# jianwen-xie/Latent-Space-Normalizing-Flow

Hardware: NVIDIA B200
Metric: langevin_latent_steps_per_sec (higher is better)
Workload: dtype fp16-hi/lo-3pass-fwd+bf16-hi/lo-3pass-bwd/f32-accumulate (fp32-equivalent)

## Files before the change

include/lsnf.h:

```cpp
#ifndef LSNF_H_
#define LSNF_H_

#include <stddef.h>
#include <stdint.h>

#ifdef __cplusplus
extern "C" {
#endif

#define LSNF_ABI_VERSION 1

typedef struct lsnf_plan lsnf_plan;
typedef void* lsnf_stream;

typedef enum lsnf_status {
  LSNF_OK = 0,
  LSNF_ERR_INVALID = -1,
  LSNF_ERR_CUDA = -2,
  LSNF_ERR_STATE = -3,
  LSNF_ERR_UNSUPPORTED = -4
} lsnf_status;

typedef enum lsnf_arch {
  LSNF_ARCH_NONE = -1,
// ... 112 lines not shown
  int32_t out_off_y[LSNF_MAX_PHASES], out_off_x[LSNF_MAX_PHASES];
  int32_t out_phase_split;
  int32_t out_channels;
  int32_t epilogue;
  int32_t k_splits;
  int32_t a_planes;
  int32_t a_h, a_w;
  int32_t tap_gen_k;
  int32_t b_k;
  int32_t b_rows;
  int32_t operand_fp16;
  int32_t passes;
  int64_t a_offset, b_offset, out_offset;
  int64_t flops;
} lsnf_stage_info;

int lsnf_plan_num_stages(const lsnf_plan* plan);
int lsnf_plan_stage_info(const lsnf_plan* plan, int32_t index, lsnf_stage_info* out);
int lsnf_plan_pack_index(const lsnf_plan* plan, int32_t index, int32_t ci, int32_t co, int32_t ky, int32_t kx,
                         int64_t* row, int64_t* col);

#define LSNF_KERNEL_SINGLE 0
#define LSNF_KERNEL_PAIR 1
typedef struct lsnf_launch_info {
  int32_t kernel;
  int32_t grid_x, grid_y, grid_z, block;
  int32_t ring_stages;
  int32_t stage_bytes;
  int32_t smem_bytes;
  int32_t ctas_per_sm;
  int32_t tmem_columns;
  int32_t tma_store;
  int32_t stream_k;
  int32_t reserved[4];
} lsnf_launch_info;
int lsnf_plan_stage_launch_info(const lsnf_plan* plan, int32_t index, int32_t num_sms, lsnf_launch_info* out);

#ifdef __cplusplus
}
#endif
#endif
```

latent-space-normalizing-flow_b200/_cabi.py:

```python
from __future__ import annotations

import ctypes as C
import os

_HERE = os.path.dirname(os.path.abspath(__file__))
LIB_PATH = os.environ.get("LSNF_LIB") or os.path.join(_HERE, "_lib", "liblsnf_b200.so")
_lib = None

LSNF_MAX_TAPS = 16
LSNF_MAX_PHASES = 4
FLOW_PTRS_PER_STEP = 12

ARCH = {"none": -1, "svhn": 0, "cifar10": 1, "celeba_crop": 2, "celeba_hq256": 3}
GEMM_TCGEN05, GEMM_SIMT = 0, 1


class Config(C.Structure):
    _fields_ = [("arch", C.c_int32), ("batch", C.c_int32), ("nz", C.c_int32), ("ngf", C.c_int32), ("nc", C.c_int32),
                ("f_depth", C.c_int32), ("f_width", C.c_int32), ("f_permutation", C.c_int32),
                ("f_coupling", C.c_int32), ("leak", C.c_float), ("gemm_impl", C.c_int32),
                ("bwd_passes", C.c_int32), ("train", C.c_int32), ("reserved", C.c_int32 * 3)]


class Tap(C.Structure):
    _fields_ = [("dy", C.c_int32), ("dx", C.c_int32), ("plane", C.c_int32), ("brow", C.c_int32)]


class StageInfo(C.Structure):
    _fields_ = [("kind", C.c_int32), ("layer", C.c_int32), ("grid_h", C.c_int32), ("grid_w", C.c_int32),
                ("box_b", C.c_int32), ("box_h", C.c_int32), ("box_w", C.c_int32), ("k_per_tap", C.c_int32),
                ("n_valid", C.c_int32), ("n_pad", C.c_int32), ("block_n", C.c_int32), ("n_phases", C.c_int32),
                ("n_taps", C.c_int32 * LSNF_MAX_PHASES), ("taps", (Tap * LSNF_MAX_TAPS) * LSNF_MAX_PHASES),
                ("out_mul", C.c_int32), ("out_off_y", C.c_int32 * LSNF_MAX_PHASES),
                ("out_off_x", C.c_int32 * LSNF_MAX_PHASES), ("out_phase_split", C.c_int32),
                ("out_channels", C.c_int32), ("epilogue", C.c_int32), ("k_splits", C.c_int32),
                ("a_planes", C.c_int32), ("a_h", C.c_int32), ("a_w", C.c_int32), ("tap_gen_k", C.c_int32),
                ("b_k", C.c_int32), ("b_rows", C.c_int32), ("operand_fp16", C.c_int32), ("passes", C.c_int32),
                ("a_offset", C.c_int64), ("b_offset", C.c_int64), ("out_offset", C.c_int64), ("flops", C.c_int64)]


class LaunchInfo(C.Structure):
    _fields_ = [("kernel", C.c_int32), ("grid_x", C.c_int32), ("grid_y", C.c_int32), ("grid_z", C.c_int32),
                ("block", C.c_int32), ("ring_stages", C.c_int32), ("stage_bytes", C.c_int32),
                ("smem_bytes", C.c_int32), ("ctas_per_sm", C.c_int32), ("tmem_columns", C.c_int32),
                ("tma_store", C.c_int32), ("stream_k", C.c_int32), ("reserved", C.c_int32 * 4)]


KERNEL_SINGLE, KERNEL_PAIR = 0, 1

EXPORTS = {
    "lsnf_abi_version": (C.c_int, []),
    "lsnf_last_error": (C.c_char_p, []),
    "lsnf_plan_create": (C.c_int, [C.POINTER(Config), C.POINTER(C.c_void_p)]),
    "lsnf_plan_destroy": (None, [C.c_void_p]),
    "lsnf_workspace_bytes": (C.c_size_t, [C.c_void_p]),
    "lsnf_plan_bind": (C.c_int, [C.c_void_p, C.c_void_p, C.c_size_t]),
    "lsnf_pack_generator_weights": (C.c_int, [C.c_void_p, C.POINTER(C.c_void_p), C.POINTER(C.c_void_p), C.c_int32,
                                              C.c_void_p]),
    "lsnf_pack_flow_weights": (C.c_int, [C.c_void_p, C.POINTER(C.c_void_p), C.POINTER(C.c_void_p),
                                         C.POINTER(C.c_void_p), C.c_void_p, C.POINTER(C.c_void_p), C.c_void_p]),
    "lsnf_generator_forward": (C.c_int, [C.c_void_p, C.c_void_p, C.c_void_p, C.c_void_p]),
    "lsnf_generator_dgrad": (C.c_int, [C.c_void_p, C.c_void_p, C.c_float, C.c_void_p, C.c_void_p]),
    "lsnf_flow_forward": (C.c_int, [C.c_void_p, C.c_void_p, C.c_void_p, C.c_void_p, C.c_void_p, C.c_void_p,
                                    C.c_void_p]),
    "lsnf_flow_inverse": (C.c_int, [C.c_void_p, C.c_void_p, C.c_void_p, C.c_void_p, C.c_void_p]),
    "lsnf_langevin_update": (C.c_int, [C.c_void_p, C.c_void_p, C.c_void_p, C.c_void_p, C.c_float, C.c_void_p,
                                       C.c_int32, C.c_uint64, C.c_uint64, C.c_uint32, C.c_void_p, C.c_void_p]),
    "lsnf_langevin_run": (C.c_int, [C.c_void_p, C.c_void_p, C.c_void_p, C.c_int32, C.c_float, C.c_float, C.c_int32,
                                    C.c_void_p, C.c_uint64, C.c_uint64, C.c_void_p, C.c_void_p, C.c_void_p]),
    "lsnf_sample_prior": (C.c_int, [C.c_void_p, C.c_void_p, C.c_void_p, C.c_void_p, C.c_int32, C.c_void_p]),
    "lsnf_generator_grad_floats": (C.c_size_t, [C.c_void_p]),
    "lsnf_generator_grad_layout": (C.c_int, [C.c_void_p, C.POINTER(C.c_int64), C.POINTER(C.c_int64)]),
    "lsnf_generator_param_grads": (C.c_int, [C.c_void_p, C.c_void_p, C.c_void_p, C.c_int32, C.c_void_p, C.c_void_p,
                                             C.c_int32, C.c_void_p]),
    "lsnf_flow_grad_floats": (C.c_size_t, [C.c_void_p]),
    "lsnf_flow_grad_layout": (C.c_int, [C.c_void_p, C.POINTER(C.c_int64), C.POINTER(C.c_int64)]),
    "lsnf_flow_param_grads": (C.c_int, [C.c_void_p, C.c_void_p, C.c_int32, C.c_void_p, C.c_void_p, C.c_void_p]),
    "lsnf_langevin_run_masked": (C.c_int, [C.c_void_p, C.c_void_p, C.c_void_p, C.c_void_p, C.c_int32, C.c_float,
# ... 53 lines not shown
```

latent-space-normalizing-flow_b200/csrc/lsnf_internal.cuh:

```cuda
#pragma once
#include <cuda.h>
#include <cuda_bf16.h>
#include <cuda_fp16.h>
#include <cuda_runtime.h>
#include <stdint.h>

#include <string>
#include <vector>

#include "lsnf.h"

namespace lsnf {

constexpr int BLOCK_M = 128;
constexpr int BLOCK_K = 64;

enum Epilogue : int32_t {
  EPI_ACT_HL = 0,
  EPI_OUT_TANH = 1,
  EPI_GRAD_HL = 2,
  EPI_PARTIAL = 3
};

struct TapDev {
  int16_t dy, dx, plane;
  int16_t bsh;
  int32_t brow;
};

struct PhaseDev {
  int32_t ntaps;
  int32_t mo, no;
  TapDev taps[LSNF_MAX_TAPS];
};

struct StageDev {
  const __nv_bfloat16* a;
  const __nv_bfloat16* b;
  int32_t aP, B, Hg, Wg, Ka, b_rows;
  int32_t aH, aW, tap_gen, b_k;
  int32_t bB, bH, bW;
  int32_t tiles_b, tiles_h, tiles_w;
  int32_t n_valid, n_pad, block_n;
  int32_t nphase, ksplit, it_per_split;
  int32_t epi, bias_mod, oC, ms, split;
  float leak;
  const float* bias;
  void* out;
  uint32_t* mbits;
  int64_t sP, sB, sH, sW, sPos;
  int32_t nc, Ho, Wo, pad_;
  int32_t fp16, out_fp16;
  int32_t passes, out_single;
  const float* descale;
  int64_t rows_total;
  float* sk_slots;
  int32_t* sk_flags;
  int32_t sk_enable;
  int32_t wgrad;
  int32_t out_tma, nst;
  PhaseDev ph[LSNF_MAX_PHASES];
};

struct StageHost {
  lsnf_stage_info info;
  StageDev dev;
  CUtensorMap tmA, tmB, tmO;
  bool maps_ready = false;
  int layer = 0;
  int kind = 0;
  int k = 0, s = 0, p = 0, ci = 0, co = 0;
  size_t a_off = 0, b_off = 0, out_off = 0, mbits_off = 0, bias_off = 0;
  size_t b_bytes = 0;
  bool last = false, first = false;
  int num_sms = 148;
};

struct FlowLayout {
  int nz, w, n_out, half;
  size_t an_b, an_e, an_ei, W, WT, Winv, W1, W1T, b1, e1, W2, W2T, b2, e2, W3, W3T, b3, e3, perm, perm_inv, ld_const;
  size_t step_floats;
  size_t vec_floats;
  size_t max_mat;
  size_t step_mat;
};

struct FlowStash {
  size_t y, u1, a1, a2, h, gu, gp1, gp2, gp3, gx, gl0, gl1, gl2, gl3;
  size_t layer_floats;
};

// ... 250 lines not shown
```

latent-space-normalizing-flow_b200/csrc/tapgemm_common.cuh:

```cuda
#pragma once
#include "lsnf_internal.cuh"

namespace lsnf {

struct RowCtx {
  int b, m, n;
  bool valid;
};

__device__ __forceinline__ void tile_origin(const StageDev& st, int mtile, int& b0, int& h0, int& w0) {
  const int wt = mtile % st.tiles_w, ht = (mtile / st.tiles_w) % st.tiles_h, bt = mtile / (st.tiles_w * st.tiles_h);
  b0 = bt * st.bB; h0 = ht * st.bH; w0 = wt * st.bW;
}

__device__ __forceinline__ RowCtx tile_row(const StageDev& st, int mtile, int r) {
  int b0, h0, w0;
  tile_origin(st, mtile, b0, h0, w0);
  RowCtx rc;
  rc.n = w0 + r % st.bW;
  rc.m = h0 + (r / st.bW) % st.bH;
  rc.b = b0 + r / (st.bW * st.bH);
  rc.valid = rc.b < st.B && rc.n < st.Wg;
  return rc;
}
// ... 45 lines not shown
    float v[NV];
#pragma unroll
    for (int j = 0; j < NV; ++j) v[j] = ((mw >> j) & 1u) ? acc[j] * st.leak : acc[j];
    __align__(16) uint16_t hi[NV], lo[NV];
    split_pack<NV>(v, st.out_fp16 != 0, hi, lo);
    size_t off;
    if (st.split)
      off = (size_t)((rc.m & 1) * 2 + (rc.n & 1)) * st.sP + (size_t)rc.b * st.sB + (size_t)(rc.m >> 1) * st.sH +
            (size_t)(rc.n >> 1) * st.sW;
    else
      off = (size_t)rc.b * st.sB + (size_t)rc.m * st.sH + (size_t)rc.n * st.sW;
    uint16_t* o = (uint16_t*)st.out + off + col;
    *reinterpret_cast<Vec*>(o) = *reinterpret_cast<Vec*>(hi);
    if (!st.out_single) *reinterpret_cast<Vec*>(o + st.oC) = *reinterpret_cast<Vec*>(lo);
  } else {
    const size_t row = ((size_t)rc.b * st.Hg + rc.m) * st.Wg + rc.n;
    float* o = (float*)st.out + ((size_t)split_idx * st.rows_total + row) * st.n_pad + col;
    *reinterpret_cast<float4*>(o) = make_float4(acc[0], acc[1], acc[2], acc[3]);
    if (NV == 8) *reinterpret_cast<float4*>(o + 4) = make_float4(acc[4], acc[5], acc[6], acc[7]);
  }
  return signs;
}

__device__ __forceinline__ void get_tap(const StageDev& st, int phase, int t, int& dy, int& dx, int& plane,
                                        int& brow, int& bcol) {
  if (st.tap_gen) {
    dy = t / st.tap_gen; dx = t % st.tap_gen; plane = 0; brow = 0; bcol = t * st.Ka;
  } else {
    const TapDev& tp = st.ph[phase].taps[t];
    dy = tp.dy; dx = tp.dx; plane = tp.plane; brow = tp.brow; bcol = tp.bsh;
  }
}

}
```

latent-space-normalizing-flow_b200/csrc/tapgemm_tc.cu:

```cuda
#include <algorithm>
#include <mutex>
#include <type_traits>

#include "tapgemm_common.cuh"

namespace lsnf {

constexpr int TC_EPI_WARPS = 8;
constexpr int TC_THREADS = 64 + 32 * TC_EPI_WARPS;
constexpr int A_TILE_BYTES = BLOCK_M * BLOCK_K * 2;
constexpr uint64_t L2_EVICT_FIRST = 0x12F0000000000000ull;
constexpr uint64_t L2_EVICT_LAST = 0x14F0000000000000ull;

constexpr int TC_MAX_STAGES = 8;
constexpr int TC_SMEM_EXTRA = 1024  + 256 ;
constexpr int TC_SMEM_MAX = 232448;
template <int BN>
struct TcCfg {
  static constexpr int B_TILE_BYTES = BN * BLOCK_K * 2;
  static constexpr int SPAN = BN >= 64 ? BN / 2 : BN;
  static constexpr int TMEM_COLS = BN < 32 ? 32 : BN;
  static constexpr bool TMA_EPI = BN >= 128;
};

// ... 224 lines not shown
          split16(t, out16, hi[q], lo[q]);
          signs |= (uint32_t)(hi[q] >> 15) << ((j + q) & 31);
        }
        *reinterpret_cast<uint4*>(o16 + cc + j) = *reinterpret_cast<uint4*>(hi);
        *reinterpret_cast<uint4*>(o16 + lo_off + cc + j) = *reinterpret_cast<uint4*>(lo);
      } else if (epi == EPI_GRAD_HL) {
        const uint32_t mw = mword >> ((cc + j) & 31);
        __align__(16) uint16_t hi[8], lo[8];
#pragma unroll
        for (int q = 0; q < 8; ++q) {
          const float t = ((mw >> q) & 1u) ? f[q] * leak : f[q];
          split16(t, out16, hi[q], lo[q]);
        }
        *reinterpret_cast<uint4*>(o16 + cc + j) = *reinterpret_cast<uint4*>(hi);
        if (!st.out_single) *reinterpret_cast<uint4*>(o16 + lo_off + cc + j) = *reinterpret_cast<uint4*>(lo);
      } else {
        *reinterpret_cast<float4*>(o32 + cc + j) = make_float4(f[0], f[1], f[2], f[3]);
        *reinterpret_cast<float4*>(o32 + cc + j + 4) = make_float4(f[4], f[5], f[6], f[7]);
      }
    }
    if constexpr (CH == 32) {
      if (epi == EPI_ACT_HL) obits[cc >> 5] = signs;
    }
  }
  if (sk_mode == 2) {
    __syncwarp();
    if (lane == 0)
      for (int h = sk_first; h < sk_self; h += sk_stride) st.sk_flags[h * TC_EPI_WARPS + ewarp] = 0;
  }
}

template <int BN, bool SINGLE>
__device__ __forceinline__ void tc_epilogue_tma(const StageDev& st, const CUtensorMap* tmO, uint32_t stage_smem,
                                                int mtile, int n0, int phase, int warp, int lane, uint32_t tmem_acc,
                                                uint32_t full_bar, uint32_t parity, int sk_mode, int sk_self,
                                                int sk_first);

template <int BN>
__global__ void __launch_bounds__(TC_THREADS, 2)
tapgemm_tc_kernel(const __grid_constant__ CUtensorMap tmA, const __grid_constant__ CUtensorMap tmB,
                  const __grid_constant__ CUtensorMap tmO, const __grid_constant__ StageDev st) {
  using Cfg = TcCfg<BN>;
  extern __shared__ uint8_t smem_raw[];
  const uint32_t tiles = (smem_u32(smem_raw) + 1023u) & ~1023u;
  const bool three = st.passes != 1;
  const uint32_t nst = (uint32_t)st.nst;
  const uint32_t a_bytes = three ? 2 * A_TILE_BYTES : A_TILE_BYTES;
  const uint32_t stage_bytes = a_bytes + (three ? 2 : 1) * Cfg::B_TILE_BYTES;
  const uint32_t bars = tiles + nst * stage_bytes;
  auto full_bar = [&](int s) { return bars + 8u * s; };
  auto empty_bar = [&](int s) { return bars + 8u * (TC_MAX_STAGES + s); };
  const uint32_t tmem_full_bar = bars + 8u * (2 * TC_MAX_STAGES);
  const uint32_t tmem_slot = bars + 8u * (2 * TC_MAX_STAGES + 1);
  uint8_t* gen_base = smem_raw + (tiles - smem_u32(smem_raw));
  volatile uint32_t* tmem_slot_ptr =
      reinterpret_cast<volatile uint32_t*>(gen_base + nst * stage_bytes + 8 * (2 * TC_MAX_STAGES + 1));

  const int warp = threadIdx.x >> 5, lane = threadIdx.x & 31;
  const int mtile = blockIdx.x, n0 = blockIdx.y * BN;
  const int zphase = blockIdx.z / st.ksplit, split = blockIdx.z % st.ksplit;
  const bool wg = st.wgrad != 0;
  const int phase = wg ? 0 : zphase, tap0 = wg ? zphase : 0;
  const int kblocks = st.Ka / BLOCK_K;
  const int total = (wg ? 1 : st.ph[phase].ntaps) * kblocks;
  const int it0 = split * st.it_per_split, it1 = min(total, it0 + st.it_per_split);

  if (warp == 0 && lane == 0) {
    asm volatile("prefetch.tensormap [%0];" ::"l"(&tmA) : "memory");
    asm volatile("prefetch.tensormap [%0];" ::"l"(&tmB) : "memory");
// ... 49 lines not shown
  } else if (warp == 1) {
    {
      const uint32_t idesc = umma_idesc<BN>(st.fp16 != 0);
      uint32_t s = 0, par = 0, sa = tiles;
      for (int it = it0; it < it1; ++it) {
        mbar_wait(full_bar(s), par);
        asm volatile("tcgen05.fence::after_thread_sync;" ::: "memory");
        const uint64_t da = umma_desc(sa), db = umma_desc(sa + a_bytes);
        if (elect_one()) {
#pragma unroll
          for (int k = 0; k < BLOCK_K / 16; ++k) {
            const uint64_t a_hi = da + 2 * k, a_lo = a_hi + (A_TILE_BYTES >> 4);
            const uint64_t b_hi = db + 2 * k, b_lo = b_hi + (Cfg::B_TILE_BYTES >> 4);
            if (three) {
              umma_bf16(tmem_base, a_lo, b_hi, idesc, (it > it0 || k > 0) ? 1u : 0u);
              umma_bf16(tmem_base, a_hi, b_lo, idesc, 1u);
              umma_bf16(tmem_base, a_hi, b_hi, idesc, 1u);
            } else {
              umma_bf16(tmem_base, a_hi, b_hi, idesc, (it > it0 || k > 0) ? 1u : 0u);
            }
          }
          umma_commit(empty_bar(s));
        }
        sa += stage_bytes;
        if (++s == nst) { s = 0; par ^= 1u; sa = tiles; }
      }
      if (elect_one()) umma_commit(tmem_full_bar);
    }
  } else {
    bool done = false;
    if constexpr (Cfg::TMA_EPI) {
      if (st.out_tma) {
        if (st.out_single)
          tc_epilogue_tma<BN, true>(st, &tmO, tiles, mtile, n0, phase, warp, lane, tmem_base, tmem_full_bar, 0u, 0, 0, 0);
        else
          tc_epilogue_tma<BN, false>(st, &tmO, tiles, mtile, n0, phase, warp, lane, tmem_base, tmem_full_bar, 0u, 0, 0, 0);
        if (warp == 2 && lane == 0) asm volatile("cp.async.bulk.wait_group 0;" ::: "memory");
        done = true;
      }
    }
    if (!done) tc_epilogue<BN>(st, mtile, n0, phase, wg ? (int)blockIdx.z : split, warp, lane, tmem_base, tmem_full_bar,
                               0u, it1 > it0);
  }
  asm volatile("tcgen05.fence::before_thread_sync;" ::: "memory");
  __syncthreads();
  if (warp == 1) {
    asm volatile("tcgen05.dealloc.cta_group::1.sync.aligned.b32 %0, %1;" ::"r"(tmem_base),
                 "r"((uint32_t)Cfg::TMEM_COLS)
                 : "memory");
  }
}

constexpr int P_BN = 256;
constexpr int P_B_TILE_BYTES = (P_BN / 2) * BLOCK_K * 2;
constexpr int P_STAGE_BYTES = 2 * A_TILE_BYTES + 2 * P_B_TILE_BYTES;
constexpr int P_STAGES = 3;
constexpr int P_MAX_STAGES = 2 * P_STAGES;
constexpr int P_EPI_STAGING = 2 * BLOCK_M * 128;
constexpr int P_SMEM_BYTES = P_STAGES * P_STAGE_BYTES + P_EPI_STAGING + 1024 + 256;
constexpr uint32_t PEER_BIT_MASK = 0xFEFFFFFFu;

__device__ __forceinline__ void tma2_load_5d(uint32_t dst, const CUtensorMap* map, uint32_t bar, int c0, int c1, int c2,
                                             int c3, int c4) {
  asm volatile(
      "cp.async.bulk.tensor.5d.cta_group::2.shared::cluster.global.mbarrier::complete_tx::bytes.L2::cache_hint [%0], [%1, {%3, %4, %5, %6, %7}], [%2], %8;"
      ::"r"(dst), "l"(map), "r"(bar), "r"(c0), "r"(c1), "r"(c2), "r"(c3), "r"(c4), "l"(L2_EVICT_LAST)
      : "memory");
}
__device__ __forceinline__ void tma2_load_2d(uint32_t dst, const CUtensorMap* map, uint32_t bar, int c0, int c1) {
// ... 16 lines not shown
      "tcgen05.commit.cta_group::2.mbarrier::arrive::one.shared::cluster.multicast::cluster.b64 [%0], %1;" ::"r"(bar),
      "h"((uint16_t)3)
      : "memory");
}
__device__ __forceinline__ void cluster_sync_all() {
  asm volatile("barrier.cluster.arrive.release.aligned;" ::: "memory");
  asm volatile("barrier.cluster.wait.acquire.aligned;" ::: "memory");
}

__device__ __forceinline__ void cluster_sync_relaxed() {
  asm volatile("barrier.cluster.arrive.relaxed.aligned;" ::: "memory");
  asm volatile("barrier.cluster.wait.aligned;" ::: "memory");
}
__device__ __forceinline__ void mbar_arrive_leader(uint32_t bar) {
  asm volatile("mbarrier.arrive.release.cluster.shared::cluster.b64 _, [%0];" ::"r"(bar & PEER_BIT_MASK) : "memory");
}

__device__ __forceinline__ void tma_store_5d(const CUtensorMap* map, uint32_t src, int c0, int c1, int c2, int c3,
                                             int c4) {
  asm volatile(
      "cp.async.bulk.tensor.5d.global.shared::cta.bulk_group.L2::cache_hint [%0, {%2, %3, %4, %5, %6}], [%1], %7;" ::"l"(map),
      "r"(src), "r"(c0), "r"(c1), "r"(c2), "r"(c3), "r"(c4), "l"(L2_EVICT_FIRST)
      : "memory");
}

__device__ __forceinline__ uint32_t pack2_16(float a, float b, bool fp16) {
  if (fp16) { const __half2 h = __floats2half2_rn(a, b); return *reinterpret_cast<const uint32_t*>(&h); }
  const __nv_bfloat162 h = __floats2bfloat162_rn(a, b);
  return *reinterpret_cast<const uint32_t*>(&h);
}

template <int BN, bool SINGLE>
__device__ __forceinline__ void tc_epilogue_tma(const StageDev& st, const CUtensorMap* tmO, uint32_t stage_smem,
                                                int mtile, int n0, int phase, int warp, int lane, uint32_t tmem_acc,
                                                uint32_t full_bar, uint32_t parity, int sk_mode, int sk_self,
                                                int sk_first) {
  const int quarter = warp & 3;
  const int half = (warp - 2) >> 2;
  const int ewarp = warp - 2;
  const int r = quarter * 32 + lane;
  const RowCtx rc = tile_row(st, mtile, r);
  const int epi = st.epi;
  const float leak = st.leak;
  const bool out16 = st.out_fp16 != 0;
  constexpr int NCH = BN / 64;
  uint32_t mb[NCH];
  uint32_t* obits = nullptr;
#pragma unroll
  for (int ch = 0; ch < NCH; ++ch) mb[ch] = 0u;
  if (epi == EPI_GRAD_HL && rc.valid) {
    const uint32_t* mrow = grad_bits_row(st, rc) + (n0 >> 5) + half;
#pragma unroll
    for (int ch = 0; ch < NCH; ++ch) mb[ch] = __ldg(mrow + 2 * ch);
  } else if (epi == EPI_ACT_HL && rc.valid) {
    const int pos = n0 / st.oC;
    const int mo = rc.m * st.ms + st.ph[phase].mo, no = rc.n * st.ms + st.ph[phase].no;
    const size_t off = (size_t)rc.b * st.sB + (size_t)mo * st.sH + (size_t)no * st.sW + (size_t)pos * st.sPos;
    obits = act_bits_word(st, off, n0 % st.oC) + half;
  }
  int b0, h0, w0;
  tile_origin(st, mtile, b0, h0, w0);
  const int cb = n0 % st.oC;
  int c1, c2, c3, c4;
  if (st.out_tma == 1) { c1 = st.ph[phase].no; c2 = w0; c3 = st.ph[phase].mo; c4 = b0 * st.Hg + h0; }
  else if (st.out_tma == 2) { c1 = n0 / st.oC; c2 = 0; c3 = 0; c4 = b0; }
  else if (st.out_tma == 3) { c1 = w0; c2 = h0; c3 = b0; c4 = 0; }
  else { c1 = w0 >> 1; c2 = b0 * (st.Hg >> 1) + (h0 >> 1); c3 = 0; c4 = 0; }
  int srow = r;
  if (st.out_tma == 4) {
    const int nl = r % st.bW, ml = (r / st.bW) % st.bH, bl = r / (st.bW * st.bH);
    srow = (((ml & 1) * 2 + (nl & 1)) * (st.bB * (st.bH >> 1)) + bl * (st.bH >> 1) + (ml >> 1)) * (st.bW >> 1) + (nl >> 1);
  }
  const float* bias = (epi == EPI_ACT_HL) ? st.bias + cb + half * 32 : nullptr;
  const float descale = st.descale ? __ldg(st.descale) : 1.f;
  const uint32_t buf0 = stage_smem, buf1 = stage_smem + 128 * 128;

  mbar_wait(full_bar, parity);
  asm volatile("tcgen05.fence::after_thread_sync;" ::: "memory");
  if (sk_mode == 2) {
    if (lane == 0) {
      for (int h = sk_first; h < sk_self; h += 2) {
        const int32_t* flag = st.sk_flags + h * TC_EPI_WARPS + ewarp;
        int32_t f;
        do {
          asm volatile("ld.acquire.gpu.global.s32 %0, [%1];" : "=r"(f) : "l"(flag) : "memory");
        } while (f == 0);
      }
    }
    __syncwarp();
    __threadfence();
  }
#pragma unroll 1
  for (int ch = 0; ch < NCH; ++ch) {
    const int col = ch * 64 + half * 32;
    uint32_t v[32];
    tmem_ld32(tmem_acc + ((uint32_t)(quarter * 32) << 16) + (uint32_t)col, v);
    asm volatile("tcgen05.wait::ld.sync.aligned;" ::: "memory");
    if (sk_mode == 2) {
      for (int h = sk_first; h < sk_self; h += 2) {
        const float* slot = st.sk_slots + ((size_t)h * 256 + col) * BLOCK_M + r;
#pragma unroll
        for (int j = 0; j < 32; ++j)
          v[j] = __float_as_uint(__uint_as_float(v[j]) + __ldcg(slot + (size_t)j * BLOCK_M));
      }
    }
    const uint32_t hi_buf = SINGLE ? ((ch & 1) ? buf1 : buf0) : buf0;
    const uint32_t lo_buf = buf1;
    if (SINGLE && warp == 2 && lane == 0) asm volatile("cp.async.bulk.wait_group.read 1;" ::: "memory");
    epi_bar_sync();
    uint32_t signs = 0u;
#pragma unroll
    for (int j = 0; j < 32; j += 8) {
      float t[8];
      if (epi == EPI_ACT_HL) {
        const float4 q0 = __ldg(reinterpret_cast<const float4*>(bias + ch * 64 + j));
        const float4 q1 = __ldg(reinterpret_cast<const float4*>(bias + ch * 64 + j + 4));
        const float bb[8] = {q0.x, q0.y, q0.z, q0.w, q1.x, q1.y, q1.z, q1.w};
#pragma unroll
        for (int q = 0; q < 8; ++q) {
          const float a = __uint_as_float(v[j + q]) * descale + bb[q];
          t[q] = a > 0.f ? a : a * leak;
          signs |= (__float_as_uint(t[q]) >> 31) << (j + q);
        }
      } else {
        const uint32_t mw = pick_word(mb, ch) >> j;
#pragma unroll
// ... 10 lines not shown
                     "r"(pack2_16(t[6], t[7], out16))
                     : "memory");
      } else {
        __align__(16) uint16_t hi[8], lo[8];
#pragma unroll
        for (int q = 0; q < 8; ++q) split16(t[q], out16, hi[q], lo[q]);
        asm volatile("st.shared.v4.b32 [%0], {%1, %2, %3, %4};" ::"r"(hi_buf + off), "r"(((uint32_t*)hi)[0]),
                     "r"(((uint32_t*)hi)[1]), "r"(((uint32_t*)hi)[2]), "r"(((uint32_t*)hi)[3])
                     : "memory");
        if (!st.out_single)
          asm volatile("st.shared.v4.b32 [%0], {%1, %2, %3, %4};" ::"r"(lo_buf + off), "r"(((uint32_t*)lo)[0]),
                       "r"(((uint32_t*)lo)[1]), "r"(((uint32_t*)lo)[2]), "r"(((uint32_t*)lo)[3])
                       : "memory");
      }
    }
    asm volatile("fence.proxy.async.shared::cta;" ::: "memory");
    epi_bar_sync();
    if (warp == 2 && lane == 0) {
      const int c0 = cb + ch * 64;
      tma_store_5d(tmO, hi_buf, c0, c1, c2, c3, c4);
      if (!SINGLE && !st.out_single) tma_store_5d(tmO, lo_buf, c0 + st.oC, c1, c2, c3, c4);
      asm volatile("cp.async.bulk.commit_group;" ::: "memory");
      if (!SINGLE) asm volatile("cp.async.bulk.wait_group.read 0;" ::: "memory");
    }
    if (obits) obits[2 * ch] = signs;
  }
  if (sk_mode == 2) {
    __syncwarp();
    if (lane == 0)
      for (int h = sk_first; h < sk_self; h += 2) st.sk_flags[h * TC_EPI_WARPS + ewarp] = 0;
  }
}

struct SkItem { int tile, ka, kb, mode; };
struct SkPlan {
  int total, t_lo, t_hi, ka_lo, kb_hi, first_fin, last_help, first_help_only, n_items, full_lo, full_hi;
  long long u0, u1;
  int strided, pair_, npairs_;
  __device__ __forceinline__ void init(int pair, int num_pairs, int num_tiles, int total_, bool stream_k) {
    total = total_;
    strided = !stream_k; pair_ = pair; npairs_ = num_pairs;
    if (strided) {
      n_items = pair < num_tiles ? (num_tiles - pair + num_pairs - 1) / num_pairs : 0;
      first_fin = last_help = first_help_only = 0;
      return;
    }
    const long long U = (long long)num_tiles * total;
    u0 = U * pair / num_pairs; u1 = U * (pair + 1) / num_pairs;
    n_items = 0; first_fin = last_help = first_help_only = 0; full_lo = 0; full_hi = -1;
    if (u1 <= u0) return;
    t_lo = (int)(u0 / total); t_hi = (int)((u1 - 1) / total);
    ka_lo = (int)(u0 - (long long)t_lo * total);
    kb_hi = (int)(u1 - (long long)t_hi * total);
    const bool first_cut = ka_lo != 0, last_cut = kb_hi != total;
    if (t_lo == t_hi) {
      if (last_cut) { last_help = 1; }
      else if (first_cut) { first_fin = 1; }
      else { full_lo = full_hi = t_lo; }
    } else {
      last_help = last_cut; first_fin = first_cut;
      full_lo = first_cut ? t_lo + 1 : t_lo;
      full_hi = last_cut ? t_hi - 1 : t_hi;
    }
    n_items = last_help + (full_hi >= full_lo ? full_hi - full_lo + 1 : 0) + first_fin;
  }
  __device__ __forceinline__ SkItem item(int j) const {
    SkItem it;
    if (strided) { it.tile = pair_ + j * npairs_; it.ka = 0; it.kb = total; it.mode = 0; return it; }
    if (last_help) {
      if (j == 0) { it.tile = t_hi; it.ka = (t_lo == t_hi) ? ka_lo : 0; it.kb = kb_hi; it.mode = 1; return it; }
      --j;
    }
    const int nfull = full_hi >= full_lo ? full_hi - full_lo + 1 : 0;
    if (j < nfull) { it.tile = full_lo + j; it.ka = 0; it.kb = total; it.mode = 0; return it; }
    it.tile = t_lo; it.ka = ka_lo; it.kb = total; it.mode = 2;
    return it;
  }
};

__device__ __forceinline__ int sk_pair_of(long long u, long long U, int P) {
  int p = (int)((u * P) / U);
  while (p > 0 && U * p / P > u) --p;
  while (p + 1 < P && U * (p + 1) / P <= u) ++p;
  return p;
}

template <bool DEEP>
__global__ void __cluster_dims__(2, 1, 1) __launch_bounds__(TC_THREADS, 1)
tapgemm_tc2_kernel(const __grid_constant__ CUtensorMap tmA, const __grid_constant__ CUtensorMap tmB,
                   const __grid_constant__ CUtensorMap tmO, const __grid_constant__ StageDev st) {
  extern __shared__ uint8_t smem_raw[];
  const uint32_t tiles = (smem_u32(smem_raw) + 1023u) & ~1023u;
  const uint32_t stage_smem = tiles + P_STAGES * P_STAGE_BYTES;
  const uint32_t bars = stage_smem + P_EPI_STAGING;
  auto full_bar = [&](int s) { return bars + 8u * s; };
  auto empty_bar = [&](int s) { return bars + 8u * (P_MAX_STAGES + s); };
  auto tmem_full_bar = [&](int a) { return bars + 8u * (2 * P_MAX_STAGES + a); };
  auto tmem_empty_bar = [&](int a) { return bars + 8u * (2 * P_MAX_STAGES + 2 + a); };
  const uint32_t tmem_slot = bars + 8u * (2 * P_MAX_STAGES + 4);
  uint8_t* gen_base = smem_raw + (tiles - smem_u32(smem_raw));
  volatile uint32_t* tmem_slot_ptr = reinterpret_cast<volatile uint32_t*>(
      gen_base + P_STAGES * P_STAGE_BYTES + P_EPI_STAGING + 8 * (2 * P_MAX_STAGES + 4));
  constexpr bool three = !DEEP;
  constexpr uint32_t nst = DEEP ? P_MAX_STAGES : P_STAGES;
  constexpr uint32_t stage_bytes = DEEP ? P_STAGE_BYTES / 2 : P_STAGE_BYTES;
  constexpr uint32_t b_off = DEEP ? A_TILE_BYTES : 2 * A_TILE_BYTES;

  uint32_t cta_rank;
  asm volatile("mov.u32 %0, %%cluster_ctarank;" : "=r"(cta_rank));
  const bool leader = cta_rank == 0;
  const int warp = threadIdx.x >> 5, lane = threadIdx.x & 31;
  const int kblocks = st.Ka / BLOCK_K;
  const int mtiles = st.tiles_b * st.tiles_h * st.tiles_w;
  const int m_pairs = (mtiles + 1) >> 1, n_tiles = st.n_pad / P_BN;
  const int num_tiles = m_pairs * n_tiles * st.nphase;
  const int pair_id = blockIdx.x >> 1, num_pairs = gridDim.x >> 1;
  const int total = st.ph[0].ntaps * kblocks;
  SkPlan sk;
  sk.init(pair_id, num_pairs, num_tiles, total, st.sk_enable != 0);

  if (warp == 0 && lane == 0) {
    asm volatile("prefetch.tensormap [%0];" ::"l"(&tmA) : "memory");
    asm volatile("prefetch.tensormap [%0];" ::"l"(&tmB) : "memory");
    if (st.out_tma) asm volatile("prefetch.tensormap [%0];" ::"l"(&tmO) : "memory");
    for (int s = 0; s < P_MAX_STAGES; ++s) {
      mbar_init(full_bar(s), 1);
      mbar_init(empty_bar(s), 1);
    }
    for (int a = 0; a < 2; ++a) {
      mbar_init(tmem_full_bar(a), 1);
      mbar_init(tmem_empty_bar(a), 2 * TC_EPI_WARPS);
    }
    asm volatile("fence.mbarrier_init.release.cluster;" ::: "memory");
  }
  if (warp == 1) {
    asm volatile("tcgen05.alloc.cta_group::2.sync.aligned.shared::cta.b32 [%0], %1;" ::"r"(tmem_slot), "r"(512u)
                 : "memory");
    asm volatile("tcgen05.relinquish_alloc_permit.cta_group::2.sync.aligned;" ::: "memory");
  }
  asm volatile("tcgen05.fence::before_thread_sync;" ::: "memory");
  __syncthreads();
  cluster_sync_all();
  asm volatile("tcgen05.fence::after_thread_sync;" ::: "memory");
  const uint32_t tmem_base = *tmem_slot_ptr;
  pdl_wait();
  pdl_trigger();

  if (warp == 0) {
    {
      uint32_t s = 0, par = 0, sa = tiles;
      constexpr uint32_t tx_bytes = three ? 2 * P_STAGE_BYTES : P_STAGE_BYTES;
      for (int j = 0; j < sk.n_items; ++j) {
        const SkItem w = sk.item(j);
        const int t = w.tile;
        const int mp = t % m_pairs, nt = (t / m_pairs) % n_tiles, phase = t / (m_pairs * n_tiles);
        const int mtile = 2 * mp + (int)cta_rank;
        int b0, h0, w0;
        tile_origin(st, mtile, b0, h0, w0);
        const int nb = nt * P_BN + (int)cta_rank * (P_BN / 2);
        int tp = w.ka / kblocks, kc = (w.ka - tp * kblocks) * BLOCK_K;
        int dy, dx, plane, brow, bcol;
        get_tap(st, phase, tp, dy, dx, plane, brow, bcol);
        for (int it = w.ka; it < w.kb; ++it) {
          mbar_wait(empty_bar(s), par ^ 1u);
          const uint32_t sb = sa + b_off;
          const uint32_t fb = full_bar(s) & PEER_BIT_MASK;
          if (elect_one()) {
            if (leader) mbar_expect_tx(full_bar(s), tx_bytes);
            tma2_load_5d(sa, &tmA, fb, kc, w0 + dx, h0 + dy, b0, plane);
            if (three) tma2_load_5d(sa + A_TILE_BYTES, &tmA, fb, st.Ka + kc, w0 + dx, h0 + dy, b0, plane);
            tma2_load_2d(sb, &tmB, fb, bcol + kc, brow + nb);
            if (three) tma2_load_2d(sb + P_B_TILE_BYTES, &tmB, fb, st.b_k + bcol + kc, brow + nb);
          }
          kc += BLOCK_K;
          if (kc == st.Ka) {
            kc = 0; ++tp;
            if (it + 1 < w.kb) get_tap(st, phase, tp, dy, dx, plane, brow, bcol);
          }
          sa += stage_bytes;
          if (++s == nst) { s = 0; par ^= 1u; sa = tiles; }
        }
      }
    }
  } else if (warp == 1) {
    if (leader) {
      const uint32_t fmt = st.fp16 ? 0u : 1u;
      const uint32_t idesc = (1u << 4) | (fmt << 7) | (fmt << 10) | ((uint32_t)(P_BN >> 3) << 17) | ((uint32_t)(256 >> 4) << 24);
      uint32_t s = 0, par = 0, sa = tiles;
      for (int j = 0; j < sk.n_items; ++j) {
        const SkItem w = sk.item(j);
        const uint32_t acc = (uint32_t)j & 1u;
        mbar_wait(tmem_empty_bar(acc), (((uint32_t)j >> 1) & 1u) ^ 1u);
        asm volatile("tcgen05.fence::after_thread_sync;" ::: "memory");
        const uint32_t d_tmem = tmem_base + acc * P_BN;
        for (int it = w.ka; it < w.kb; ++it) {
          mbar_wait(full_bar(s), par);
          asm volatile("tcgen05.fence::after_thread_sync;" ::: "memory");
          const uint64_t da = umma_desc(sa), db = umma_desc(sa + b_off);
          if (elect_one()) {
#pragma unroll
            for (int k = 0; k < BLOCK_K / 16; ++k) {
              const uint64_t a_hi = da + 2 * k, a_lo = a_hi + (A_TILE_BYTES >> 4);
              const uint64_t b_hi = db + 2 * k, b_lo = b_hi + (P_B_TILE_BYTES >> 4);
              if (three) {
                umma2_bf16(d_tmem, a_lo, b_hi, idesc, (it > w.ka || k > 0) ? 1u : 0u);
                umma2_bf16(d_tmem, a_hi, b_lo, idesc, 1u);
                umma2_bf16(d_tmem, a_hi, b_hi, idesc, 1u);
              } else {
                umma2_bf16(d_tmem, a_hi, b_hi, idesc, (it > w.ka || k > 0) ? 1u : 0u);
              }
            }
            umma2_commit_both(empty_bar(s));
          }
          sa += stage_bytes;
          if (++s == nst) { s = 0; par ^= 1u; sa = tiles; }
        }
        if (elect_one()) umma2_commit_both(tmem_full_bar(acc));
      }
    }
  } else {
    const long long U = (long long)num_tiles * total;
    for (int j = 0; j < sk.n_items; ++j) {
      const SkItem w = sk.item(j);
      const int t = w.tile;
      const int mp = t % m_pairs, nt = (t / m_pairs) % n_tiles, phase = t / (m_pairs * n_tiles);
      const int mtile = 2 * mp + (int)cta_rank;
      const uint32_t acc = (uint32_t)j & 1u;
      const int self = 2 * pair_id + (int)cta_rank;
      int first = self;
      if (w.mode == 2) first = 2 * sk_pair_of((long long)t * total, U, num_pairs) + (int)cta_rank;
      if (st.out_tma && w.mode != 1) {
        if (st.out_single)
          tc_epilogue_tma<P_BN, true>(st, &tmO, stage_smem, mtile, nt * P_BN, phase, warp, lane,
                                      tmem_base + acc * P_BN, tmem_full_bar(acc), ((uint32_t)j >> 1) & 1u, w.mode,
                                      self, first);
        else
          tc_epilogue_tma<P_BN, false>(st, &tmO, stage_smem, mtile, nt * P_BN, phase, warp, lane,
                                       tmem_base + acc * P_BN, tmem_full_bar(acc), ((uint32_t)j >> 1) & 1u, w.mode,
                                       self, first);
      } else
        tc_epilogue<P_BN>(st, mtile, nt * P_BN, phase, 0, warp, lane, tmem_base + acc * P_BN, tmem_full_bar(acc),
                          ((uint32_t)j >> 1) & 1u, true, w.mode, self, first, 2);
      asm volatile("tcgen05.fence::before_thread_sync;" ::: "memory");
      __syncwarp();
      if (lane == 0) mbar_arrive_leader(tmem_empty_bar(acc));
    }
    if (st.out_tma && warp == 2 && lane == 0) asm volatile("cp.async.bulk.wait_group 0;" ::: "memory");
  }
  asm volatile("tcgen05.fence::before_thread_sync;" ::: "memory");
  __syncthreads();
  cluster_sync_relaxed();
  if (warp == 1) {
    asm volatile("tcgen05.dealloc.cta_group::2.sync.aligned.b32 %0, %1;" ::"r"(tmem_base), "r"(512u) : "memory");
  }
}

typedef CUresult (*EncodeTiledFn)(CUtensorMap*, CUtensorMapDataType, cuuint32_t, void*, const cuuint64_t*,
                                  const cuuint64_t*, const cuuint32_t*, const cuuint32_t*, CUtensorMapInterleave,
                                  CUtensorMapSwizzle, CUtensorMapL2promotion, CUtensorMapFloatOOBfill);

static EncodeTiledFn get_encode() {
  static EncodeTiledFn fn = nullptr;
  if (fn) return fn;
  void* p = nullptr;
  cudaDriverEntryPointQueryResult q;
  if (cudaGetDriverEntryPoint("cuTensorMapEncodeTiled", &p, cudaEnableDefault, &q) != cudaSuccess ||
      q != cudaDriverEntryPointSuccess)
    return nullptr;
  fn = (EncodeTiledFn)p;
  return fn;
// ... 99 lines not shown
      const cuuint64_t plane = (cuuint64_t)d.B * Hh * Wh * C2;
      dims[0] = C2; dims[1] = Wh; dims[2] = (cuuint64_t)d.B * Hh; dims[3] = 2; dims[4] = 2;
      strides[0] = C2 * eb; strides[1] = Wh * C2 * eb; strides[2] = plane * eb; strides[3] = 2 * plane * eb;
      box[0] = 64; box[1] = d.bW / 2; box[2] = d.bB * d.bH / 2; box[3] = 2; box[4] = 2;
      kind = 4;
    }
    if (kind) {
      CUresult r = enc(&sh.tmO, CU_TENSOR_MAP_DATA_TYPE_BFLOAT16, 5, d.out, dims, strides, box, es,
                       CU_TENSOR_MAP_INTERLEAVE_NONE, CU_TENSOR_MAP_SWIZZLE_128B, CU_TENSOR_MAP_L2_PROMOTION_NONE,
                       CU_TENSOR_MAP_FLOAT_OOB_FILL_NONE);
      if (r != CUDA_SUCCESS) {
        set_error("cuTensorMapEncodeTiled(out) failed with code " + std::to_string((int)r) + " for stage layer " +
                  std::to_string(sh.layer) + " kind " + std::to_string(sh.kind));
        return LSNF_ERR_CUDA;
      }
      sh.dev.out_tma = kind;
    }
  }
  if (!sh.dev.out_tma) sh.tmO = sh.tmA;
  sh.maps_ready = true;
  return LSNF_OK;
}

template <int BN>
static int launch_bn(const StageHost& sh, cudaStream_t s) {
  StageDev st = sh.dev;
  const RingGeom g = ring_geometry(st);
  st.nst = g.nst;
  dim3 grid(st.tiles_b * st.tiles_h * st.tiles_w, st.n_pad / BN, (st.wgrad ? st.ph[0].ntaps : st.nphase) * st.ksplit);
  LSNF_CUDA(launch_k(tapgemm_tc_kernel<BN>, grid, dim3(TC_THREADS), g.smem, s, sh.tmA, sh.tmB, sh.tmO, st));
  return LSNF_OK;
}

static bool pair_stream_k(const StageDev& st, int max_pairs) {
  const int mtiles = st.tiles_b * st.tiles_h * st.tiles_w;
  const int num_tiles = (mtiles + 1) / 2 * (st.n_pad / P_BN) * st.nphase;
  const int total = st.ph[0].ntaps * (st.Ka / BLOCK_K);
  const int rounds = (num_tiles + max_pairs - 1) / max_pairs;
  const long long static_units = (long long)rounds * total;
  const long long sk_units = ((long long)num_tiles * total + max_pairs - 1) / max_pairs + 35;
  return sk_units < static_units && total >= 8 &&
         (long long)num_tiles * total >= 4LL * max_pairs && max_pairs <= 80;
}

static int launch_pair(const StageHost& sh, cudaStream_t s) {
  const StageDev& st = sh.dev;
  const int mtiles = st.tiles_b * st.tiles_h * st.tiles_w;
  const int num_tiles = (mtiles + 1) / 2 * (st.n_pad / P_BN) * st.nphase;
  const int max_pairs = sh.num_sms / 2;
  StageDev launch_st = st;
  launch_st.sk_enable = pair_stream_k(st, max_pairs);
  const int pairs = launch_st.sk_enable ? max_pairs : std::min(num_tiles, max_pairs);
  dim3 grid(2 * pairs, 1, 1);
  if (st.passes == 1)
    LSNF_CUDA(launch_k(tapgemm_tc2_kernel<true>, grid, dim3(TC_THREADS), P_SMEM_BYTES, s, sh.tmA, sh.tmB, sh.tmO, launch_st));
  else
    LSNF_CUDA(launch_k(tapgemm_tc2_kernel<false>, grid, dim3(TC_THREADS), P_SMEM_BYTES, s, sh.tmA, sh.tmB, sh.tmO, launch_st));
  return LSNF_OK;
}

void tc_launch_info(const StageHost& sh_in, int num_sms, lsnf_launch_info* out) {
  StageHost sh = sh_in;
  sh.dev.out_tma = out_tma_kind(sh);
  const StageDev& d = sh.dev;
  const int mtiles = d.tiles_b * d.tiles_h * d.tiles_w;
  memset(out, 0, sizeof(*out));
  out->block = TC_THREADS;
  out->tma_store = d.out_tma;
  out->tmem_columns = use_pair(sh) ? 512 : (d.block_n < 32 ? 32 : d.block_n);
  if (use_pair(sh)) {
    const int max_pairs = num_sms / 2;
    const int num_tiles = (mtiles + 1) / 2 * (d.n_pad / P_BN) * d.nphase;
    out->kernel = LSNF_KERNEL_PAIR;
    out->stream_k = pair_stream_k(d, max_pairs) ? 1 : 0;
    out->grid_x = 2 * (out->stream_k ? max_pairs : std::min(num_tiles, max_pairs));
    out->grid_y = out->grid_z = 1;
    out->ring_stages = d.passes == 1 ? P_MAX_STAGES : P_STAGES;
    out->stage_bytes = d.passes == 1 ? P_STAGE_BYTES / 2 : P_STAGE_BYTES;
    out->smem_bytes = P_SMEM_BYTES;
    out->ctas_per_sm = 1;
  } else {
    const RingGeom g = ring_geometry(d);
    out->kernel = LSNF_KERNEL_SINGLE;
    out->grid_x = mtiles; out->grid_y = d.n_pad / d.block_n; out->grid_z = d.nphase * d.ksplit;
    out->ring_stages = g.nst;
    out->stage_bytes = (int32_t)g.stage_bytes;
    out->smem_bytes = (int32_t)g.smem;
    const int by_smem = (TC_SMEM_MAX + 1024) / ((int)g.smem + 1024);
    out->ctas_per_sm = std::max(1, std::min(by_smem, 2048 / TC_THREADS));
  }
}

int tc_prepare_device(int device) {
  static std::mutex mu;
  static bool done[64] = {false};
  std::lock_guard<std::mutex> lock(mu);
  if (device < 0 || device >= 64) { set_error("device index out of range"); return LSNF_ERR_INVALID; }
  if (done[device]) return LSNF_OK;
  LSNF_CUDA(cudaFuncSetAttribute(tapgemm_tc_kernel<256>, cudaFuncAttributeMaxDynamicSharedMemorySize, TC_SMEM_MAX));
  LSNF_CUDA(cudaFuncSetAttribute(tapgemm_tc_kernel<128>, cudaFuncAttributeMaxDynamicSharedMemorySize, TC_SMEM_MAX));
  LSNF_CUDA(cudaFuncSetAttribute(tapgemm_tc_kernel<64>, cudaFuncAttributeMaxDynamicSharedMemorySize, TC_SMEM_MAX));
  LSNF_CUDA(cudaFuncSetAttribute(tapgemm_tc_kernel<32>, cudaFuncAttributeMaxDynamicSharedMemorySize, TC_SMEM_MAX));
  LSNF_CUDA(cudaFuncSetAttribute(tapgemm_tc_kernel<16>, cudaFuncAttributeMaxDynamicSharedMemorySize, TC_SMEM_MAX));
  LSNF_CUDA(cudaFuncSetAttribute(tapgemm_tc2_kernel<false>, cudaFuncAttributeMaxDynamicSharedMemorySize, P_SMEM_BYTES));
  LSNF_CUDA(cudaFuncSetAttribute(tapgemm_tc2_kernel<true>, cudaFuncAttributeMaxDynamicSharedMemorySize, P_SMEM_BYTES));
  done[device] = true;
  return LSNF_OK;
}
// ... 16 lines not shown
```

Measured before the change: 92210.

## Split pair-CTA GEMM tiles into half/quarter N-width items to balance waves

New measurement: 93620, median of 6. 1.02x the previous value.

```diff
diff --git a/include/lsnf.h b/include/lsnf.h
--- a/include/lsnf.h
+++ b/include/lsnf.h
@@ -168,7 +168,8 @@
   int32_t tmem_columns;
   int32_t tma_store;
   int32_t stream_k;
-  int32_t reserved[4];
+  int32_t pair_whole, pair_half, pair_quarter;
+  int32_t reserved[1];
 } lsnf_launch_info;
 int lsnf_plan_stage_launch_info(const lsnf_plan* plan, int32_t index, int32_t num_sms, lsnf_launch_info* out);
 
diff --git a/latent-space-normalizing-flow_b200/_cabi.py b/latent-space-normalizing-flow_b200/_cabi.py
--- a/latent-space-normalizing-flow_b200/_cabi.py
+++ b/latent-space-normalizing-flow_b200/_cabi.py
@@ -43,7 +43,8 @@
     _fields_ = [("kernel", C.c_int32), ("grid_x", C.c_int32), ("grid_y", C.c_int32), ("grid_z", C.c_int32),
                 ("block", C.c_int32), ("ring_stages", C.c_int32), ("stage_bytes", C.c_int32),
                 ("smem_bytes", C.c_int32), ("ctas_per_sm", C.c_int32), ("tmem_columns", C.c_int32),
-                ("tma_store", C.c_int32), ("stream_k", C.c_int32), ("reserved", C.c_int32 * 4)]
+                ("tma_store", C.c_int32), ("stream_k", C.c_int32), ("pair_whole", C.c_int32),
+                ("pair_half", C.c_int32), ("pair_quarter", C.c_int32), ("reserved", C.c_int32 * 1)]
 
 
 KERNEL_SINGLE, KERNEL_PAIR = 0, 1
diff --git a/latent-space-normalizing-flow_b200/csrc/lsnf_internal.cuh b/latent-space-normalizing-flow_b200/csrc/lsnf_internal.cuh
--- a/latent-space-normalizing-flow_b200/csrc/lsnf_internal.cuh
+++ b/latent-space-normalizing-flow_b200/csrc/lsnf_internal.cuh
@@ -32,6 +32,11 @@
   int32_t ntaps;
   int32_t mo, no;
   TapDev taps[LSNF_MAX_TAPS];
+};
+
+struct PairSched {
+  int32_t stream_k;
+  int32_t whole, half, quarter;
 };
 
 struct StageDev {
@@ -56,7 +61,7 @@
   int64_t rows_total;
   float* sk_slots;
   int32_t* sk_flags;
-  int32_t sk_enable;
+  PairSched pair;
   int32_t wgrad;
   int32_t out_tma, nst;
   PhaseDev ph[LSNF_MAX_PHASES];
diff --git a/latent-space-normalizing-flow_b200/csrc/tapgemm_common.cuh b/latent-space-normalizing-flow_b200/csrc/tapgemm_common.cuh
--- a/latent-space-normalizing-flow_b200/csrc/tapgemm_common.cuh
+++ b/latent-space-normalizing-flow_b200/csrc/tapgemm_common.cuh
@@ -101,4 +101,42 @@
   }
 }
 
+__host__ __device__ __forceinline__ void pair_item(const PairSched& s, int g, int& tile, int& col, int& width) {
+  if (g < s.whole) { tile = g; col = 0; width = 256; return; }
+  g -= s.whole;
+  if (g < 2 * s.half) { tile = s.whole + (g >> 1); col = (g & 1) * 128; width = 128; return; }
+  g -= 2 * s.half;
+  tile = s.whole + s.half + (g >> 2); col = (g & 3) * 64; width = 64;
 }
+__host__ __device__ __forceinline__ int pair_items(const PairSched& s) { return s.whole + 2 * s.half + 4 * s.quarter; }
+
+constexpr int PAIR_COST_HALF = 600, PAIR_COST_QUARTER = 450;
+constexpr int PAIR_SK_ROUND_TRIP = 35;
+
+inline long long pair_critical_path(const PairSched& s, int tiles, int kblocks, int pairs) {
+  if (s.stream_k) return ((long long)tiles * kblocks + pairs - 1) / pairs * 1000 + PAIR_SK_ROUND_TRIP * 1000LL;
+  auto firsts = [pairs](int lo, int hi) { return (hi + pairs - 1) / pairs - (lo + pairs - 1) / pairs; };
+  const int h0 = s.whole, q0 = h0 + 2 * s.half, end = q0 + 4 * s.quarter;
+  return (long long)kblocks *
+         (1000LL * firsts(0, h0) + (long long)PAIR_COST_HALF * firsts(h0, q0) + (long long)PAIR_COST_QUARTER * firsts(q0, end));
+}
+
+inline PairSched pair_schedule(int tiles, int kblocks, int pairs, bool narrow) {
+  PairSched best = {0, tiles, 0, 0};
+  long long best_cp = pair_critical_path(best, tiles, kblocks, pairs);
+  const PairSched sk = {1, 0, 0, 0};
+  if (kblocks >= 8 && (long long)tiles * kblocks >= 4LL * pairs && pairs <= 80 &&
+      pair_critical_path(sk, tiles, kblocks, pairs) < best_cp)
+    return sk;
+  if (narrow) {
+    for (int whole = tiles; whole >= 0 && whole >= (tiles / pairs - 1) * pairs; --whole)
+      for (int half = tiles - whole; half >= 0; --half) {
+        const PairSched c = {0, whole, half, tiles - whole - half};
+        const long long cp = pair_critical_path(c, tiles, kblocks, pairs);
+        if (cp < best_cp) { best = c; best_cp = cp; }
+      }
+  }
+  return best;
+}
+
+}
diff --git a/latent-space-normalizing-flow_b200/csrc/tapgemm_tc.cu b/latent-space-normalizing-flow_b200/csrc/tapgemm_tc.cu
--- a/latent-space-normalizing-flow_b200/csrc/tapgemm_tc.cu
+++ b/latent-space-normalizing-flow_b200/csrc/tapgemm_tc.cu
@@ -280,9 +280,9 @@
 
 template <int BN, bool SINGLE>
 __device__ __forceinline__ void tc_epilogue_tma(const StageDev& st, const CUtensorMap* tmO, uint32_t stage_smem,
-                                                int mtile, int n0, int phase, int warp, int lane, uint32_t tmem_acc,
-                                                uint32_t full_bar, uint32_t parity, int sk_mode, int sk_self,
-                                                int sk_first);
+                                                int mtile, int n0, int width, int phase, int warp, int lane,
+                                                uint32_t tmem_acc, uint32_t full_bar, uint32_t parity, int sk_mode,
+                                                int sk_self, int sk_first);
 
 template <int BN>
 __global__ void __launch_bounds__(TC_THREADS, 2)
@@ -398,9 +398,9 @@
     if constexpr (Cfg::TMA_EPI) {
       if (st.out_tma) {
         if (st.out_single)
-          tc_epilogue_tma<BN, true>(st, &tmO, tiles, mtile, n0, phase, warp, lane, tmem_base, tmem_full_bar, 0u, 0, 0, 0);
+          tc_epilogue_tma<BN, true>(st, &tmO, tiles, mtile, n0, BN, phase, warp, lane, tmem_base, tmem_full_bar, 0u, 0, 0, 0);
         else
-          tc_epilogue_tma<BN, false>(st, &tmO, tiles, mtile, n0, phase, warp, lane, tmem_base, tmem_full_bar, 0u, 0, 0, 0);
+          tc_epilogue_tma<BN, false>(st, &tmO, tiles, mtile, n0, BN, phase, warp, lane, tmem_base, tmem_full_bar, 0u, 0, 0, 0);
         if (warp == 2 && lane == 0) asm volatile("cp.async.bulk.wait_group 0;" ::: "memory");
         done = true;
       }
@@ -483,9 +483,9 @@
 
 template <int BN, bool SINGLE>
 __device__ __forceinline__ void tc_epilogue_tma(const StageDev& st, const CUtensorMap* tmO, uint32_t stage_smem,
-                                                int mtile, int n0, int phase, int warp, int lane, uint32_t tmem_acc,
-                                                uint32_t full_bar, uint32_t parity, int sk_mode, int sk_self,
-                                                int sk_first) {
+                                                int mtile, int n0, int width, int phase, int warp, int lane,
+                                                uint32_t tmem_acc, uint32_t full_bar, uint32_t parity, int sk_mode,
+                                                int sk_self, int sk_first) {
   const int quarter = warp & 3;
   const int half = (warp - 2) >> 2;
   const int ewarp = warp - 2;
@@ -495,6 +495,7 @@
   const float leak = st.leak;
   const bool out16 = st.out_fp16 != 0;
   constexpr int NCH = BN / 64;
+  const int nch = width / 64;
   uint32_t mb[NCH];
   uint32_t* obits = nullptr;
 #pragma unroll
@@ -502,7 +503,8 @@
   if (epi == EPI_GRAD_HL && rc.valid) {
     const uint32_t* mrow = grad_bits_row(st, rc) + (n0 >> 5) + half;
 #pragma unroll
-    for (int ch = 0; ch < NCH; ++ch) mb[ch] = __ldg(mrow + 2 * ch);
+    for (int ch = 0; ch < NCH; ++ch)
+      if (ch < nch) mb[ch] = __ldg(mrow + 2 * ch);
   } else if (epi == EPI_ACT_HL && rc.valid) {
     const int pos = n0 / st.oC;
     const int mo = rc.m * st.ms + st.ph[phase].mo, no = rc.n * st.ms + st.ph[phase].no;
@@ -542,7 +544,7 @@
     __threadfence();
   }
 #pragma unroll 1
-  for (int ch = 0; ch < NCH; ++ch) {
+  for (int ch = 0; ch < nch; ++ch) {
     const int col = ch * 64 + half * 32;
     uint32_t v[32];
     tmem_ld32(tmem_acc + ((uint32_t)(quarter * 32) << 16) + (uint32_t)col, v);
@@ -619,16 +621,18 @@
   }
 }
 
-struct SkItem { int tile, ka, kb, mode; };
+struct SkItem { int tile, ka, kb, mode, col, width; };
 struct SkPlan {
   int total, t_lo, t_hi, ka_lo, kb_hi, first_fin, last_help, first_help_only, n_items, full_lo, full_hi;
   long long u0, u1;
   int strided, pair_, npairs_;
-  __device__ __forceinline__ void init(int pair, int num_pairs, int num_tiles, int total_, bool stream_k) {
+  PairSched ps;
+  __device__ __forceinline__ void init(int pair, int num_pairs, int num_tiles, int total_, const PairSched& sched) {
     total = total_;
-    strided = !stream_k; pair_ = pair; npairs_ = num_pairs;
+    strided = !sched.stream_k; pair_ = pair; npairs_ = num_pairs; ps = sched;
     if (strided) {
-      n_items = pair < num_tiles ? (num_tiles - pair + num_pairs - 1) / num_pairs : 0;
+      const int n = pair_items(sched);
+      n_items = pair < n ? (n - pair + num_pairs - 1) / num_pairs : 0;
       first_fin = last_help = first_help_only = 0;
       return;
     }
@@ -653,7 +657,12 @@
   }
   __device__ __forceinline__ SkItem item(int j) const {
     SkItem it;
-    if (strided) { it.tile = pair_ + j * npairs_; it.ka = 0; it.kb = total; it.mode = 0; return it; }
+    it.col = 0; it.width = P_BN;
+    if (strided) {
+      pair_item(ps, pair_ + j * npairs_, it.tile, it.col, it.width);
+      it.ka = 0; it.kb = total; it.mode = 0;
+      return it;
+    }
     if (last_help) {
       if (j == 0) { it.tile = t_hi; it.ka = (t_lo == t_hi) ? ka_lo : 0; it.kb = kb_hi; it.mode = 1; return it; }
       --j;
@@ -704,7 +713,7 @@
   const int pair_id = blockIdx.x >> 1, num_pairs = gridDim.x >> 1;
   const int total = st.ph[0].ntaps * kblocks;
   SkPlan sk;
-  sk.init(pair_id, num_pairs, num_tiles, total, st.sk_enable != 0);
+  sk.init(pair_id, num_pairs, num_tiles, total, st.pair);
 
   if (warp == 0 && lane == 0) {
     asm volatile("prefetch.tensormap [%0];" ::"l"(&tmA) : "memory");
@@ -744,7 +753,7 @@
         const int mtile = 2 * mp + (int)cta_rank;
         int b0, h0, w0;
         tile_origin(st, mtile, b0, h0, w0);
-        const int nb = nt * P_BN + (int)cta_rank * (P_BN / 2);
+        const int nb = nt * P_BN + w.col + (int)cta_rank * (w.width / 2);
         int tp = w.ka / kblocks, kc = (w.ka - tp * kblocks) * BLOCK_K;
         int dy, dx, plane, brow, bcol;
         get_tap(st, phase, tp, dy, dx, plane, brow, bcol);
@@ -772,7 +781,7 @@
   } else if (warp == 1) {
     if (leader) {
       const uint32_t fmt = st.fp16 ? 0u : 1u;
-      const uint32_t idesc = (1u << 4) | (fmt << 7) | (fmt << 10) | ((uint32_t)(P_BN >> 3) << 17) | ((uint32_t)(256 >> 4) << 24);
+      const uint32_t idesc0 = (1u << 4) | (fmt << 7) | (fmt << 10) | ((uint32_t)(256 >> 4) << 24);
       uint32_t s = 0, par = 0, sa = tiles;
       for (int j = 0; j < sk.n_items; ++j) {
         const SkItem w = sk.item(j);
@@ -780,6 +789,7 @@
         mbar_wait(tmem_empty_bar(acc), (((uint32_t)j >> 1) & 1u) ^ 1u);
         asm volatile("tcgen05.fence::after_thread_sync;" ::: "memory");
         const uint32_t d_tmem = tmem_base + acc * P_BN;
+        const uint32_t idesc = idesc0 | ((uint32_t)(w.width >> 3) << 17);
         for (int it = w.ka; it < w.kb; ++it) {
           mbar_wait(full_bar(s), par);
           asm volatile("tcgen05.fence::after_thread_sync;" ::: "memory");
@@ -818,11 +828,11 @@
       if (w.mode == 2) first = 2 * sk_pair_of((long long)t * total, U, num_pairs) + (int)cta_rank;
       if (st.out_tma && w.mode != 1) {
         if (st.out_single)
-          tc_epilogue_tma<P_BN, true>(st, &tmO, stage_smem, mtile, nt * P_BN, phase, warp, lane,
+          tc_epilogue_tma<P_BN, true>(st, &tmO, stage_smem, mtile, nt * P_BN + w.col, w.width, phase, warp, lane,
                                       tmem_base + acc * P_BN, tmem_full_bar(acc), ((uint32_t)j >> 1) & 1u, w.mode,
                                       self, first);
         else
-          tc_epilogue_tma<P_BN, false>(st, &tmO, stage_smem, mtile, nt * P_BN, phase, warp, lane,
+          tc_epilogue_tma<P_BN, false>(st, &tmO, stage_smem, mtile, nt * P_BN + w.col, w.width, phase, warp, lane,
                                        tmem_base + acc * P_BN, tmem_full_bar(acc), ((uint32_t)j >> 1) & 1u, w.mode,
                                        self, first);
       } else
@@ -988,27 +998,20 @@
   return LSNF_OK;
 }
 
-static bool pair_stream_k(const StageDev& st, int max_pairs) {
+static PairSched pair_sched(const StageDev& st, int max_pairs, int* pairs) {
   const int mtiles = st.tiles_b * st.tiles_h * st.tiles_w;
   const int num_tiles = (mtiles + 1) / 2 * (st.n_pad / P_BN) * st.nphase;
-  const int total = st.ph[0].ntaps * (st.Ka / BLOCK_K);
-  const int rounds = (num_tiles + max_pairs - 1) / max_pairs;
-  const long long static_units = (long long)rounds * total;
-  const long long sk_units = ((long long)num_tiles * total + max_pairs - 1) / max_pairs + 35;
-  return sk_units < static_units && total >= 8 &&
-         (long long)num_tiles * total >= 4LL * max_pairs && max_pairs <= 80;
+  const PairSched ps = pair_schedule(num_tiles, st.ph[0].ntaps * (st.Ka / BLOCK_K), max_pairs, st.out_tma != 0);
+  *pairs = ps.stream_k ? max_pairs : std::min(pair_items(ps), max_pairs);
+  return ps;
 }
 
 static int launch_pair(const StageHost& sh, cudaStream_t s) {
-  const StageDev& st = sh.dev;
-  const int mtiles = st.tiles_b * st.tiles_h * st.tiles_w;
-  const int num_tiles = (mtiles + 1) / 2 * (st.n_pad / P_BN) * st.nphase;
-  const int max_pairs = sh.num_sms / 2;
-  StageDev launch_st = st;
-  launch_st.sk_enable = pair_stream_k(st, max_pairs);
-  const int pairs = launch_st.sk_enable ? max_pairs : std::min(num_tiles, max_pairs);
+  StageDev launch_st = sh.dev;
+  int pairs;
+  launch_st.pair = pair_sched(sh.dev, sh.num_sms / 2, &pairs);
   dim3 grid(2 * pairs, 1, 1);
-  if (st.passes == 1)
+  if (launch_st.passes == 1)
     LSNF_CUDA(launch_k(tapgemm_tc2_kernel<true>, grid, dim3(TC_THREADS), P_SMEM_BYTES, s, sh.tmA, sh.tmB, sh.tmO, launch_st));
   else
     LSNF_CUDA(launch_k(tapgemm_tc2_kernel<false>, grid, dim3(TC_THREADS), P_SMEM_BYTES, s, sh.tmA, sh.tmB, sh.tmO, launch_st));
@@ -1025,11 +1028,12 @@
   out->tma_store = d.out_tma;
   out->tmem_columns = use_pair(sh) ? 512 : (d.block_n < 32 ? 32 : d.block_n);
   if (use_pair(sh)) {
-    const int max_pairs = num_sms / 2;
-    const int num_tiles = (mtiles + 1) / 2 * (d.n_pad / P_BN) * d.nphase;
+    int pairs;
+    const PairSched ps = pair_sched(d, num_sms / 2, &pairs);
     out->kernel = LSNF_KERNEL_PAIR;
-    out->stream_k = pair_stream_k(d, max_pairs) ? 1 : 0;
-    out->grid_x = 2 * (out->stream_k ? max_pairs : std::min(num_tiles, max_pairs));
+    out->stream_k = ps.stream_k;
+    out->pair_whole = ps.whole; out->pair_half = ps.half; out->pair_quarter = ps.quarter;
+    out->grid_x = 2 * pairs;
     out->grid_y = out->grid_z = 1;
     out->ring_stages = d.passes == 1 ? P_MAX_STAGES : P_STAGES;
     out->stage_bytes = d.passes == 1 ? P_STAGE_BYTES / 2 : P_STAGE_BYTES;
```
